# mmdagent/distantspeechrecognition-mirror

Hardware: AMD Instinct MI355X
Metric: decoded_audio_hours_per_sec (higher is better)
Workload: dtype f32

## Files before the change

### distantspeechrecognition-mirror_amd/csrc/k_viterbi.hip

```cpp
#include "common.h"
#include "wfst_graph.h"
#include "lattice.h"
#include "lexicon.h"
#include "wordtrace.h"
#include <algorithm>
#include <cmath>
#include <type_traits>

namespace dsr {

struct Tok { int32_t node; float ac; float lm; uint32_t bp; };
struct TokA { float ac; float lm; uint32_t bp; uint32_t xs; };
struct TokB { int32_t node; int32_t cnt; };
struct XRecD { int32_t dist; float cost; uint32_t meta; float eps1; int32_t dst; int32_t p2; int32_t dstXoff; int32_t dstCnt; };
struct Side { double ttl; float ac; float lm; int32_t rec; uint32_t prevBp; int32_t c; uint32_t next; };
struct CandA { double ttl; float ac; float lm; };
struct CandB { int32_t dst; int32_t next; int32_t rec; uint32_t prevBp; };
struct Bp { uint32_t prev; uint32_t rec; };

static constexpr uint32_t kNone = 0xFFFFFFFFu;
static constexpr uint32_t kEndBit = 0x80000000u;
static constexpr int kThreads = 1024;
static constexpr int kWaves = kThreads / 64;
static constexpr int kFastK = 8;
static constexpr int kB = 2;
static constexpr int kFastC = 24576;
static constexpr int kFastE = 8190;
static constexpr int kP1 = 16;
static constexpr int kW = 4;
static constexpr int kProfN = 48;
static constexpr int kSideLds = 496;

struct GraphDev {
  int nNodes, initial;
  const int* xoff; const XRec* xrec; const XRecD* xrecD; const int* xarc; const int* xpathOff;
  const int* eoff; const ERec* erec; const int* path; const float* pathCost;
  const float* arcCost; const uint32_t* arcOut; const uint32_t* arcIn;
  const int* nodeFinal; const float* nodeCost;
};

struct SegState { int n, status, maxActive, pad; long arenaOff, chunkEnd, arenaUsed; double thresh; long long stat[3]; };

struct DecDev {
  double beam, lmScale, lmPenalty, silPenalty; uint32_t silenceX; int noPen;
  int segFrames, segCount, segQueues, segDrop; long poolCap, poolChunk;    unsigned long long* poolNext; SegState* segState; int* segDone; TokA* saveA; TokB* saveB;
  int maxTok, maxCand; long arenaCap;
  TokA* tokA; TokB* tokB; TokA* ctok; Side* side; int fastOK; int* tokOff; int* tokCnt; int* owner; int* rank; int* chead; CandA* cA; CandB* cB; unsigned* first; unsigned* tags; Bp* arena;
  int* queue; long long* prof;
  int dumpOn; long dumpCap; long* dumpFrameOff; int* dumpNode; float* dumpAc; float* dumpLm; int* dumpArc; long* dumpCount;
  int latOn; long latCap; uint4* lat; double* latTtl; long* latFrameOff; int* arenaLat; int4* latFinal; int* latInfo;
  int topN; TokA* tokA3; TokB* tokB3;
};

struct VitArgs {
  GraphDev G; DecDev D;
  const float* scores; const int* nframesArr; int U, Tmax, nDist;
  dsr_decode_result* res; int* arcsOut; unsigned* wordsOut; int maxPath, useLdsRow, hashN, regionB, cntCap;
};
typedef const __attribute__((address_space(4))) VitArgs* KP;

__device__ __forceinline__ unsigned ld_u32(const unsigned* p) { return __hip_atomic_load(p, __ATOMIC_RELAXED, __HIP_MEMORY_SCOPE_AGENT); }
__device__ __forceinline__ int ld_i32(const int* p) { return __hip_atomic_load(p, __ATOMIC_RELAXED, __HIP_MEMORY_SCOPE_AGENT); }
__device__ __forceinline__ void st_u32(unsigned* p, unsigned v) { __hip_atomic_store(p, v, __ATOMIC_RELAXED, __HIP_MEMORY_SCOPE_AGENT); }
__device__ __forceinline__ void st_i32(int* p, int v) { __hip_atomic_store(p, v, __ATOMIC_RELAXED, __HIP_MEMORY_SCOPE_AGENT); }
__device__ __forceinline__ void st_u64_dev(void* p, unsigned long long v) { __hip_atomic_store(reinterpret_cast<unsigned long long*>(p), v, __ATOMIC_RELAXED, __HIP_MEMORY_SCOPE_AGENT); }
__device__ __forceinline__ unsigned long long ld_u64_dev(const void* p) { return __hip_atomic_load(reinterpret_cast<const unsigned long long*>(p), __ATOMIC_RELAXED, __HIP_MEMORY_SCOPE_AGENT); }

__device__ __forceinline__ int wave_incl_scan(int v, int )
{
  v += __builtin_amdgcn_update_dpp(0, v, 0x111, 0xF, 0xF, true);
  v += __builtin_amdgcn_update_dpp(0, v, 0x112, 0xF, 0xF, true);
  v += __builtin_amdgcn_update_dpp(0, v, 0x114, 0xF, 0xF, true);
// ... 101 lines not shown
  unsigned* const tab = hkey; const int tabN = NARROW ? 2 * hashN : hashN;
  Side* sideL = reinterpret_cast<Side*>(hfirst + hashN);
  unsigned short* cntL = reinterpret_cast<unsigned short*>(reinterpret_cast<unsigned char*>(hfirst + hashN) + regionB);
  __shared__ int s_waveTot[kWaves];
  __shared__ int s_waveTotE[kWaves];
  __shared__ double s_waveMin[kWaves];
  __shared__ float s_waveMag[kWaves];
  __shared__ unsigned long long s_waveKey[kWaves];
  __shared__ int s_sideN;
  __shared__ int s_tb[2];
  __shared__ unsigned s_bm[kFastC / 32];
  __shared__ unsigned s_gbase[kFastC / 64 + 4];
  __shared__ int s_cnt[(kFastK + 32) * kWaves];
  __shared__ int s_err;
  __shared__ long long s_prof[32]; __shared__ long long s_tlast;
  __shared__ long long s_hist[PROF ? 12 : 1]; __shared__ long long s_tfr;
  __shared__ long long s_stat[3];
  __shared__ int s_maxActive; __shared__ unsigned s_tag; __shared__ long long s_latOff;
  if (PROF && threadIdx.x < 32) s_prof[threadIdx.x] = 0;
  if (PROF && threadIdx.x < 12) s_hist[threadIdx.x] = 0;
#define TICK(ix) do { if (PROF && tid == 0) { const long long tn = (long long) wall_clock64(); s_prof[ix] += tn - s_tlast; s_tlast = tn; } } while (0)
  constexpr int nthr = kThreads, nw = kWaves;
  __shared__ int s_u, s_seg, s_help; __shared__ long long s_chunk;

  const int tid = threadIdx.x;
  const int slot = blockIdx.x;
#define TOKA(ix) ((EXTRA && (ix) == 2) ? ka->D.tokA3 + (size_t) slot * ka->D.maxTok : ka->D.tokA + ((size_t) slot * 2 + (size_t) (ix)) * ka->D.maxTok)
#define TOKB(ix) ((EXTRA && (ix) == 2) ? ka->D.tokB3 + (size_t) slot * ka->D.maxTok : ka->D.tokB + ((size_t) slot * 2 + (size_t) (ix)) * ka->D.maxTok)
#define curA TOKA(bufCur)
#define nxtA TOKA(bufNxt)
#define curB TOKB(bufCur)
#define nxtB TOKB(bufNxt)
#define sprA TOKA(bufSpr)
#define sprB TOKB(bufSpr)
#define ctok (ka->D.ctok + (size_t) slot * 8192)
// ... 85 lines not shown
      const int mode = (fr == T) ? 1 : 0;
      if (mode == 0 && useLdsRow) {
        if (preRow) {
          if (tid < nDist) srow[tid] = rowNext[0];
          if (tid + nthr < nDist) srow[tid + nthr] = rowNext[1];
          if (fr + 1 < T) {
            const float* nr = sc + (size_t) (fr + 1) * nDist;
            if (tid < nDist) rowNext[0] = nr[tid];
            if (tid + nthr < nDist) rowNext[1] = nr[tid + nthr];
          }
        } else { for (int i = tid; i < nDist; i += nthr) srow[i] = sc[(size_t) fr * nDist + i]; }
      }
      const float* rowG = sc + (size_t) fr * nDist;
      int numNew = 0, numStat = -1;
      if (fr > 0) TICK(23);
      if (PROF && tid == 0) { s_tlast = (long long) wall_clock64(); s_tfr = s_tlast; }
      bool fast = fastOK && mode == 0 && n <= fastCapN && !(EXTRA && (ka->D.latOn || ka->D.topN > 0));
      int Cfr = 0;

      if (fast) {
        const bool pre = preC >= 0;
        const int chunkT = ((n + nw * 64 - 1) / (nw * 64)) * 64;
        int C = preC, E = n;
        if (!pre) {
        float psc[kP1]; int pcn[kP1]; unsigned pk[kP1];
        int runC = 0, runE = 0;
        {
          const int b0 = wave * chunkT, b1 = (b0 + chunkT < n) ? b0 + chunkT : n;
#pragma unroll
          for (int g = 0; g < kP1; g += 8) {
            if (g * 64 < chunkT && cntOK) {
// ... 51 lines not shown
          for (int it = 0; it < kP1; it++) if (pk[it] & 0x80000000u) {
            const int e = ebase + (int) ((pk[it] >> 15) & 0xFFFFu); const int off = cbase + (int) (pk[it] & 0x7FFFu);
            if (!ident) ctok[e] = curA[wave * chunkT + it * 64 + lane];
            atomicOr(&s_bm[off >> 5], 1u << (off & 31));
            for (int g = (off >> 6) + 1; g <= ((off + pcn[it]) >> 6); g++) s_gbase[g] = (unsigned) (e + 1) | ((unsigned) (64 * g - off) << 13);
          }
          __syncthreads();
        }
        } else __syncthreads();
        if (C > fastCapC || E > eCap || C > regC) { fast = false; __syncthreads(); }
        else {
          RELOAD();
          const bool ident = (E == n);
          const TokA* __restrict__ ctk = ident ? curA : ctok;
          TICK(1);
          Cfr = C;
          RELOAD();
          int tq = tid; asm volatile("" : "+v"(tq)); const int lq = tq & 63, wq = tq >> 6;
          const int K = (C + nthr - 1) / nthr;
          float qac[kFastK], qlm[kFastK]; int qrec[kFastK]; unsigned ek[kFastK];
          double* const ttlS = reinterpret_cast<double*>(cA);
          uint4* const ovf = reinterpret_cast<uint4*>(cB);
          const XRecD* const xrecD = ka->G.xrecD; const float* const pathCost = ka->G.pathCost; const uint32_t silenceX = ka->D.silenceX;
          double locMin = HUGE_VAL; float locMag = 0.0f;
          const bool prevNull0 = (fr == 0);
          const double lmS = ka->D.lmScale, lsPen = __dmul_rn(ka->D.lmScale, ka->D.lmPenalty), lsSil = __dmul_rn(ka->D.lmScale, ka->D.silPenalty);
          const bool sil0 = (0u == silenceX);
#pragma unroll
          for (int k = 0; k < kFastK; k++) { qac[k] = 0.0f; qlm[k] = 0.0f; qrec[k] = 0; ek[k] = 0u; }

          const int nPass = (!NARROW && C > tableC) ? 2 : 1;
          auto table_insert = [&](const unsigned dst, const unsigned prod, const int c) __attribute__((always_inline)) -> unsigned {
            const unsigned key = dst + 1u;
// ... 402 lines not shown
            auto stage1 = [&](const int k, const float ac, const float lm, const int rec, const unsigned ekk) __attribute__((always_inline)) {
              const bool isFirst = (keepMask >> k) & 1ull;
              const unsigned long long bal = __ballot(isFirst);
              if (isFirst) stage[s_cnt[k * nw + wq] + __popcll(bal & ((1ull << lq) - 1ull))] = make_uint4(__float_as_uint(ac), __float_as_uint(lm), (unsigned) rec, ekk);
            };
#pragma unroll
            for (int k = 0; k < kFastK; k++) if (k < K) stage1(k, qac[k], qlm[k], qrec[k], ek[k]);
            for (int kb = kFastK; kb < K; kb += kB) {
              float oac[kB], olm[kB]; int orec[kB]; unsigned oek[kB]; park_load(kb, oac, olm, orec, oek);
#pragma unroll
              for (int i = 0; i < kB; i++) if (kb + i < K) stage1(kb + i, oac[i], olm[i], orec[i], oek[i]);
            }
            __syncthreads();
            TICK(21);
            const int q4 = hashN >> 2;
            const bool layNext = prune && numNew <= 2 * nthr;
            preC = -1;
            for (int f0 = 0; f0 < numNew; f0 += 2 * nthr) {
              uint4 en[2]; int4 dx[2]; uint32_t pv[2];
#pragma unroll
              for (int i = 0; i < 2; i++) {
                const int f = f0 + i * nthr + tq; const bool on = f < numNew;
                en[i] = stage[on ? f : 0];
                if (on) { unsigned wv = (NARROW || f < q4) ? 0u : 0xFFFFFFFFu; asm volatile("" : "+v"(wv)); stage[f] = make_uint4(wv, wv, wv, wv); }
              }
#pragma unroll
              for (int i = 0; i < 2; i++) {
                const bool on = f0 + i * nthr + tq < numNew;
                dx[i] = *at32<int4>(xrecW, (on ? (en[i].z & 0x3FFFFFFFu) : 0u) * 32u + 16u);
                const bool sw = on && (en[i].w & 0x80000000u) != 0u; const unsigned si = en[i].w & 0x7FFFFFFFu;
                const uint32_t* pb = (sw && si >= (unsigned) sideLds) ? &side[si].prevBp : &ctk[(sw || !on) ? 0u : (en[i].w & 0x1FFFu)].bp;
                pv[i] = *pb;
                if (sw && si < (unsigned) sideLds) pv[i] = sideL[si].prevBp;
              }
              if (layNext) {
                const int cA0 = (tq < numNew) ? dx[0].w : 0, cB0 = (nthr + tq < numNew) ? dx[1].w : 0;
                const int inA = wave_incl_scan(cA0, lq), inB = wave_incl_scan(cB0, lq);
                const bool bad = (tq < numNew && cA0 == 0) || (nthr + tq < numNew && cB0 == 0);
                const int badW = __any(bad) ? 1 : 0;
                if (lq == 63) { s_waveTot[wq] = inA; s_waveTotE[wq] = inB | (badW << 30); }
                __syncthreads();
                const int ta = (lq < nw) ? s_waveTot[lq] : 0, tbv = (lq < nw) ? s_waveTotE[lq] : 0, tb = tbv & 0x3FFFFFFF;
                const int sa = wave_incl_scan(ta, lq), sb = wave_incl_scan(tb, lq);
                const int totA = __builtin_amdgcn_readlane(sa, 63), totB = __builtin_amdgcn_readlane(sb, 63), wu = uni(wq);
                const int total = totA + totB;
                const int offA = total - (__builtin_amdgcn_readlane(sa - ta, wu) + inA), offB = total - (totA + __builtin_amdgcn_readlane(sb - tb, wu) + inB);
                const bool anyBad = __any((tbv >> 30) & 1);
#pragma unroll
                for (int i = 0; i < 2; i++) {
                  const int f = i * nthr + tq; const int off = i ? offB : offA, cn = i ? cB0 : cA0;
                  if (f < numNew && cn > 0) {
                    const int e = numNew - 1 - f;
                    atomicOr(&s_bm[off >> 5], 1u << (off & 31));
                    for (int g = (off >> 6) + 1; g <= ((off + cn) >> 6); g++) s_gbase[g] = (unsigned) (e + 1) | ((unsigned) (64 * g - off) << 13);
                  }
                }
                if (tq == 0) { s_sideN = 0; s_gbase[0] = 0; s_err = 0; }
                preC = anyBad ? -1 : total;
              }
#pragma unroll
              for (int i = 0; i < 2; i++) {
                const int f = f0 + i * nthr + tq;
                if (f < numNew) {
                  const int pos = numNew - 1 - f;
                  TokA na; na.ac = __uint_as_float(en[i].x); na.lm = __uint_as_float(en[i].y); na.bp = (uint32_t) (arenaOff + pos); na.xs = (uint32_t) dx[i].z | ((en[i].z & 0x40000000u) ? 0x80000000u : 0u);
                  TokB nb; nb.node = dx[i].x; nb.cnt = dx[i].w;
                  Bp bp; bp.prev = pv[i]; bp.rec = (uint32_t) (en[i].z & 0x3FFFFFFFu);
                  outA[pos] = na; outB[pos] = nb; outBp[pos] = bp;
                  if (pos < cntCap) cntL[pos] = (unsigned short) dx[i].w;
                }
              }
            }
            TICK(22);
          } else
          {
#pragma unroll
          for (int g4 = 0; g4 < kFastK; g4 += kW) if (g4 < K) write4(std::integral_constant<int, kW>{}, g4, &qac[g4], &qlm[g4], &qrec[g4], &ek[g4]);
          for (int kb = kFastK; kb < K; kb += kB) {
            float oac[kB], olm[kB]; int orec[kB]; unsigned oek[kB]; park_load(kb, oac, olm, orec, oek);
            write4(std::integral_constant<int, kB>{}, kb, oac, olm, orec, oek);
          }
          TICK(21);
          TICK(22);
          preC = -1;
          }
          cntOK = prune && numNew <= cntCap;
// ... 223 lines not shown
        }
      }
      if (EXTRA && ka->D.latOn) {
        uint4* lat = ka->D.lat + (size_t) u * ka->D.latCap; double* ltt = ka->D.latTtl + (size_t) u * ka->D.latCap;
        const long latOff = (long) s_latOff;
        for (int c = tid; c < C; c += nthr) {
          const CandA a = cA[c]; const CandB b = cB[c];
          lat[latOff + c] = make_uint4(__float_as_uint(a.ac), __float_as_uint(a.lm), (unsigned) b.rec, b.prevBp); ltt[latOff + c] = a.ttl;
        }
        __syncthreads();
        if (tid == 0) { s_latOff = latOff + C; ka->D.latFrameOff[(size_t) u * (ka->Tmax + 3) + fr + 1] = latOff + C; }
      }
      }
      __syncthreads();
      TICK(fast ? 7 : 8);
      if (PROF && tid == 0 && mode == 0) { const int cls = !fast ? 3 : Cfr <= kFastK * nthr ? 0 : Cfr <= 12288 ? 1 : 2; s_hist[cls] += 1; s_hist[4 + cls] += s_tlast - s_tfr; s_hist[8 + cls] += Cfr; }
      RELOAD();
      if (mode == 0) {
        if (dump) {
          long* cnt = ka->D.dumpCount; const long o = cnt[0];
          if (o + numNew <= ka->D.dumpCap) {
            for (int i = tid; i < numNew; i += nthr) {
              const TokA t = ld_tok(&nxtA[i]); ka->D.dumpNode[o + i] = nxtB[i].node; ka->D.dumpAc[o + i] = t.ac; ka->D.dumpLm[o + i] = t.lm;
              ka->D.dumpArc[o + i] = ka->G.xarc[arena[t.bp].rec];
            }
          }
          __syncthreads();
          if (tid == 0) { ka->D.dumpFrameOff[fr] = o; ka->D.dumpFrameOff[fr + 1] = o + numNew; cnt[0] = o + numNew; cnt[1] = fr + 1; }
        }
        if (numStat < 0) numStat = numNew;
        if (numStat == 0 || numNew == 0) { status = DSR_E_CONSISTENCY; break; }
// ... 105 lines not shown
      else __builtin_amdgcn_fence(__ATOMIC_RELEASE, "workgroup");
      __syncthreads();
      if (tid == 0) st_i32(&ka->D.segDone[u], seg + 1);
      continue;
    }
    if (status != DSR_OK) {
      if (tid == 0) {
        dsr_decode_result* const res = ka->res; clear_result(&res[u]); res[u].status = status; res[u].frames = T - 1;
        if (segS > 0) { st_i32(&ka->D.segState[u].status, status); asm volatile("s_waitcnt vmcnt(0)" ::: "memory"); st_i32(&ka->D.segDone[u], 0x7FFFFFFF); }
      }
    }
  }
  RELOAD();
  if (tid == 0) ka->D.tags[slot] = s_tag;
  if (PROF && tid < 32) ka->D.prof[slot * kProfN + tid] = s_prof[tid];
  if (PROF && tid < 12) ka->D.prof[slot * kProfN + 32 + tid] = s_hist[tid];
#undef TICK
#undef RELOAD
#undef TOKA
#undef TOKB
#undef curA
#undef nxtA
#undef curB
#undef nxtB
#undef sprA
#undef sprB
#undef ctok
#undef side
#undef cA
#undef cB
#undef arena
// ... 7 lines not shown
  DevBuf<int> d_xoff, d_xarc, d_xpathOff, d_eoff, d_path, d_nodeFinal, d_queue; DevBuf<float> d_pathCost;
  DevBuf<XRec> d_xrec; DevBuf<ERec> d_erec; DevBuf<float> d_arcCost, d_nodeCost; DevBuf<uint32_t> d_arcOut, d_arcIn;
  DevBuf<TokA> d_tokA, d_ctok; DevBuf<TokB> d_tokB; DevBuf<Side> d_side; DevBuf<XRecD> d_xrecD; int fastOK = 0; int maxCnt = 0; DevBuf<int> d_tokOff, d_tokCnt, d_owner, d_rank, d_chead; DevBuf<unsigned> d_tags; DevBuf<CandA> d_cA; DevBuf<CandB> d_cB; DevBuf<unsigned> d_first; DevBuf<Bp> d_arena;
  DevBuf<long long> d_prof; DevBuf<dsr_decode_result> d_res; DevBuf<int> d_arcs; DevBuf<unsigned> d_words;
  long arenaCap = 0; int initial = 0; unsigned tokenMemoryLimit = 0;
  long lastPoolCap = 0;
  DevBuf<SegState> d_segState; DevBuf<int> d_segDone; DevBuf<unsigned long long> d_poolNext; DevBuf<TokA> d_saveA; DevBuf<TokB> d_saveB;
  DevBuf<WTok> w_tok; DevBuf<WCand> w_cand; DevBuf<int> w_tokOff, w_rank; DevBuf<unsigned long long> w_best; DevBuf<unsigned> w_first; DevBuf<int4> w_traces; size_t w_tablesFor = 0;
  bool costNegZero = false; double costMinAbs = HUGE_VAL;
  DevBuf<uint4> d_lat; DevBuf<double> d_latTtl; DevBuf<long> d_latFrameOff; DevBuf<int> d_arenaLat; DevBuf<int4> d_latFinal; DevBuf<int> d_latInfo;
  int latU = 0, latTmax = 0; long latArenaCap = 0; WfstGraph graphCopy; DevBuf<TokA> d_tokA3; DevBuf<TokB> d_tokB3;
  const dsr_lexicon* lexIn = nullptr; const dsr_lexicon* lexOut = nullptr; uint32_t eosX = 0; std::string eosSymbol;
  int lastU = 0; size_t lastMaxPath = 0; bool lastPaths = false;
  PinBuf<dsr_decode_result> h_res; PinBuf<int> h_arcs; PinBuf<unsigned> h_words; hipEvent_t evDone = nullptr;
  int pendingU = 0; size_t pendingPath = 0; int pendingSlots = 0; long long* pendingProf = nullptr;
  int dumpOn = 0; long dumpCap = 0; DevBuf<long> d_dumpFrameOff, d_dumpCount; DevBuf<int> d_dumpNode, d_dumpArc; DevBuf<float> d_dumpAc, d_dumpLm;
  std::vector<int64_t> h_dumpFrameOff; std::vector<int32_t> h_dumpNode, h_dumpArc; std::vector<float> h_dumpAc, h_dumpLm; int64_t h_dumpFrames = 0;
};

}

using namespace dsr;
struct dsr_wfst : WfstGraph { dsr_lexicon* lexState = nullptr; dsr_lexicon* lexIn = nullptr; dsr_lexicon* lexOut = nullptr; };
struct dsr_decoder : DecoderState {};

extern "C" {

dsr_status dsr_wfst_create(dsr_wfst** out) { return guard([&] { if (!out) throw Error(DSR_E_PARAMETER, "null argument"); *out = new dsr_wfst(); }); }
dsr_status dsr_wfst_set_sorted_output(dsr_wfst* g, int on)
{ return guard([&] { if (!g) throw Error(DSR_E_PARAMETER, "null argument"); if (!g->arcs.empty()) throw Error(DSR_E_CONSISTENCY, "the transducer already has arcs"); g->sortedOutput = on != 0; }); }
// ... 260 lines not shown
      DSR_HIP(hipMemsetAsync(d->d_queue.p, 0, 8 * sizeof(int), st));
      WtArgs A; A.nNodes = d->nNodes; A.initial = d->initial; A.xoff = d->d_xoff.p; A.xrec = d->d_xrec.p; A.xarc = d->d_xarc.p; A.xpathOff = d->d_xpathOff.p; A.eoff = d->d_eoff.p;
      A.erec = d->d_erec.p; A.path = d->d_path.p; A.arcCost = d->d_arcCost.p; A.arcOut = d->d_arcOut.p; A.arcIn = d->d_arcIn.p; A.nodeFinal = d->d_nodeFinal.p; A.nodeCost = d->d_nodeCost.p;
      A.beam = c.beam; A.lmScale = c.lmScale; A.lmPenalty = c.lmPenalty; A.silPenalty = c.silPenalty; A.silenceX = c.silenceX; A.insertSilence = c.insertSilence;
      A.maxTok = c.maxActive; A.maxCand = c.maxCandidates; A.maxTraces = maxTraces;
      A.tok = d->w_tok.p; A.cand = d->w_cand.p; A.tokOff = d->w_tokOff.p; A.rank = d->w_rank.p; A.bestKey = d->w_best.p; A.firstSlot = d->w_first.p; A.traces = d->w_traces.p; A.queue = d->d_queue.p;
      A.scores = score; A.nframes = nframes; A.U = U; A.Tmax = Tmax; A.nDist = nDist; A.res = d->d_res.p; A.arcsOut = d->d_arcs.p; A.wordsOut = d->d_words.p; A.maxPath = maxPath;
      wordtrace_launch(A, slots, st);
      const size_t nPath = want_paths ? (size_t) U * maxPath : 0;
      d->h_res.reserve(U); d->h_arcs.reserve(nPath ? nPath : 1); d->h_words.reserve(nPath ? nPath : 1);
      DSR_HIP(hipMemcpyAsync(d->h_res.p, d->d_res.p, sizeof(dsr_decode_result) * U, hipMemcpyDeviceToHost, st));
      if (nPath) DSR_HIP(hipMemcpyAsync(d->h_arcs.p, d->d_arcs.p, sizeof(int) * nPath, hipMemcpyDeviceToHost, st));
      if (nPath) DSR_HIP(hipMemcpyAsync(d->h_words.p, d->d_words.p, sizeof(unsigned) * nPath, hipMemcpyDeviceToHost, st));
      if (!d->evDone) DSR_HIP(hipEventCreateWithFlags(&d->evDone, hipEventDisableTiming));
      DSR_HIP(hipEventRecord(d->evDone, st));
      d->pendingU = U; d->pendingPath = nPath; d->pendingSlots = slots; d->pendingProf = nullptr; d->latU = 0;
      return;
    }
    int32_t* arcs_out = want_paths ? (int32_t*) 1 : nullptr; uint32_t* words_out = want_paths ? (uint32_t*) 1 : nullptr;
    for (size_t a = 0; a < d->csr.in.size(); a++) if (d->csr.in[a] > (uint32_t) nDist) throw Error(DSR_E_INDEX, "arc input %u has no distribution (nDist=%d)", d->csr.in[a], nDist);
    int slots = d->cfg.streams; if (slots > U) slots = U; if (d->dumpOn) slots = 1;
    const bool latOn = d->cfg.latticeTokens > 0;
    if (latOn && d->dumpOn) throw Error(DSR_E_PARAMETER, "lattice bookkeeping and the token dump are separate debugging aids: enable one");
    int segFrames = 0;
    if (!latOn && !d->dumpOn && d->cfg.topN <= 0 && U > slots) {
      segFrames = getenv("DSR_VITERBI_SEG") ? atoi(getenv("DSR_VITERBI_SEG")) : 125;
      if (segFrames < 0 || 2 * segFrames > Tmax + 1) segFrames = 0;
      const double saveGB = (double) U * (double) d->cfg.maxActive * 24.0 / 1e9;
      if (saveGB > (getenv("DSR_VITERBI_SEG_SAVE_GB") ? atof(getenv("DSR_VITERBI_SEG_SAVE_GB")) : 16.0)) segFrames = 0;
    }
    int segQueues = 8;
// ... 26 lines not shown
    D.silenceX = d->cfg.silenceX; D.maxTok = d->cfg.maxActive; D.maxCand = d->cfg.maxCandidates; D.arenaCap = d->arenaCap;
    D.tokA = d->d_tokA.p; D.tokB = d->d_tokB.p; D.ctok = d->d_ctok.p; D.side = d->d_side.p; D.fastOK = d->fastOK; D.tokOff = d->d_tokOff.p; D.owner = d->d_owner.p; D.rank = d->d_rank.p; D.cA = d->d_cA.p; D.cB = d->d_cB.p;
    D.first = d->d_first.p; D.tags = d->d_tags.p; D.tokCnt = d->d_tokCnt.p; D.chead = d->d_chead.p; D.arena = d->d_arena.p; D.queue = d->d_queue.p;
    D.segDrop = getenv("DSR_VITERBI_SEG_DROP") ? (int) strtol(getenv("DSR_VITERBI_SEG_DROP"), nullptr, 0) : 0;
    D.segQueues = segQueues; D.segFrames = segFrames; D.segCount = segFrames > 0 ? (Tmax + segFrames) / segFrames : 1;
    D.poolCap = 0; D.poolChunk = 0; D.poolNext = nullptr; D.segState = nullptr; D.segDone = nullptr; D.saveA = nullptr; D.saveB = nullptr;
    if (segFrames > 0) {
      d->d_segState.reserve(U); d->d_segDone.reserve(U); d->d_poolNext.reserve(1);
      d->d_saveA.reserve((size_t) U * d->cfg.maxActive); d->d_saveB.reserve((size_t) U * d->cfg.maxActive);
      DSR_HIP(hipMemsetAsync(d->d_segDone.p, 0, sizeof(int) * (size_t) U, st)); DSR_HIP(hipMemsetAsync(d->d_poolNext.p, 0, sizeof(unsigned long long), st));
      D.poolCap = (long) ((size_t) std::max(poolArenas, slots) * (size_t) d->arenaCap); if (D.poolCap > (long) 0xFFFFFFF0L) D.poolCap = (long) 0xFFFFFFF0L;
      D.poolChunk = std::min<long>(262144, std::max<long>(4096, D.poolCap / (4 * (long) U)));
      D.poolNext = d->d_poolNext.p; D.segState = d->d_segState.p; D.segDone = d->d_segDone.p; D.saveA = d->d_saveA.p; D.saveB = d->d_saveB.p;
    }
    d->lastPoolCap = D.poolCap;
    D.prof = nullptr;
    if (getenv("DSR_VITERBI_PROF")) { d->d_prof.reserve((size_t) slots * kProfN); D.prof = d->d_prof.p; }
    D.dumpOn = d->dumpOn; D.dumpCap = d->dumpCap; D.dumpFrameOff = d->d_dumpFrameOff.p; D.dumpNode = d->d_dumpNode.p; D.dumpAc = d->d_dumpAc.p;
    D.dumpLm = d->d_dumpLm.p; D.dumpArc = d->d_dumpArc.p; D.dumpCount = d->d_dumpCount.p;
    D.topN = d->cfg.topN > 0 ? d->cfg.topN : 0; D.tokA3 = nullptr; D.tokB3 = nullptr;
    if (D.topN > 0) { d->d_tokA3.reserve((size_t) slots * d->cfg.maxActive); d->d_tokB3.reserve((size_t) slots * d->cfg.maxActive); D.tokA3 = d->d_tokA3.p; D.tokB3 = d->d_tokB3.p; }
    D.latOn = latOn ? 1 : 0; D.latCap = 0; D.lat = nullptr; D.latTtl = nullptr; D.latFrameOff = nullptr; D.arenaLat = nullptr; D.latFinal = nullptr; D.latInfo = nullptr;
    if (latOn) {
      const size_t cap = (size_t) d->cfg.latticeTokens;
      d->d_lat.reserve((size_t) U * cap); d->d_latTtl.reserve((size_t) U * cap); d->d_latFrameOff.reserve((size_t) U * (Tmax + 3));
      d->d_arenaLat.reserve((size_t) U * (size_t) d->arenaCap); d->d_latFinal.reserve((size_t) U * d->cfg.maxActive); d->d_latInfo.reserve((size_t) 4 * U);
      DSR_HIP(hipMemsetAsync(d->d_latInfo.p, 0, sizeof(int) * 4 * (size_t) U, st));
      D.latCap = (long) cap; D.lat = d->d_lat.p; D.latTtl = d->d_latTtl.p; D.latFrameOff = d->d_latFrameOff.p; D.arenaLat = d->d_arenaLat.p; D.latFinal = d->d_latFinal.p; D.latInfo = d->d_latInfo.p;
      d->latU = U; d->latTmax = Tmax; d->latArenaCap = d->arenaCap;
    } else d->latU = 0;
// ... 5 lines not shown
    int useLds = (size_t) nDist * sizeof(float) <= 64 * 1024;
    if (useLds && (size_t) ((nDist + 3) & ~3) * sizeof(float) + (size_t) hashMax * 8 + eoffB > ldsCap) useLds = 0;
    const size_t rowB = useLds ? (size_t) ((nDist + 3) & ~3) * sizeof(float) : 16;
    int hashN = hashMax; while (hashN > 0 && rowB + (size_t) hashN * 8 + eoffB > ldsCap) hashN >>= 1;
    if (getenv("DSR_VITERBI_NOHASH")) hashN = 0;
    int cntCap = (hashN > 0 && d->maxCnt < 65536 && rowB + (size_t) hashN * 8 + eoffB + 4096 <= ldsCap) ? 2048 : 0;
    if (getenv("DSR_VITERBI_NOCNT")) cntCap = 0;
    const size_t lds = rowB + (size_t) hashN * 8 + eoffB + 2 * (size_t) cntCap;
    const char* const tableEnv = getenv("DSR_VITERBI_TABLE");
    const bool narrow = d->nNodes <= 65535 && hashN == hashMax && !(tableEnv && !strcmp(tableEnv, "wide"));
    if (narrow) modes |= 4;
    if (getenv("DSR_VITERBI_SEG_VERBOSE")) fprintf(stderr, "[dsr viterbi] %d utterances on %d workgroups: %s, %s state table\n", U, slots, segFrames > 0 ? (segQueues == 8 ? "time-sliced, XCD-bound queues" : "time-sliced, one queue") : "run to completion", narrow ? "narrow" : "wide");
    VitArgs A; A.G = G; A.D = D; A.scores = score; A.nframesArr = nframes; A.U = U; A.Tmax = Tmax; A.nDist = nDist; A.res = d->d_res.p;
    A.arcsOut = (arcs_out || words_out) ? d->d_arcs.p : nullptr; A.wordsOut = (arcs_out || words_out) ? d->d_words.p : nullptr; A.maxPath = maxPath;
    A.useLdsRow = useLds; A.hashN = hashN; A.regionB = (int) eoffB; A.cntCap = cntCap;
#define DSR_LAUNCH_V(MM) { DSR_HIP(hipFuncSetAttribute((const void*) k_viterbi<MM>, hipFuncAttributeMaxDynamicSharedMemorySize, (int) lds)); \
      hipLaunchKernelGGL(k_viterbi<MM>, dim3(slots), dim3(kThreads), lds, st, A); }
    switch (modes) { case 0: DSR_LAUNCH_V(0) break; case 1: DSR_LAUNCH_V(1) break; case 2: DSR_LAUNCH_V(2) break; case 3: DSR_LAUNCH_V(3) break;
                     case 4: DSR_LAUNCH_V(4) break; case 5: DSR_LAUNCH_V(5) break; case 6: DSR_LAUNCH_V(6) break; default: DSR_LAUNCH_V(7) break; }
#undef DSR_LAUNCH_V
    DSR_HIP(hipGetLastError());
    const size_t nPath = want_paths ? (size_t) U * maxPath : 0;
    d->h_res.reserve(U); d->h_arcs.reserve(nPath ? nPath : 1); d->h_words.reserve(nPath ? nPath : 1);
    DSR_HIP(hipMemcpyAsync(d->h_res.p, d->d_res.p, sizeof(dsr_decode_result) * U, hipMemcpyDeviceToHost, st));
    if (nPath) DSR_HIP(hipMemcpyAsync(d->h_arcs.p, d->d_arcs.p, sizeof(int) * nPath, hipMemcpyDeviceToHost, st));
    if (nPath) DSR_HIP(hipMemcpyAsync(d->h_words.p, d->d_words.p, sizeof(unsigned) * nPath, hipMemcpyDeviceToHost, st));
    if (!d->evDone) DSR_HIP(hipEventCreateWithFlags(&d->evDone, hipEventDisableTiming));
    DSR_HIP(hipEventRecord(d->evDone, st));
    d->pendingU = U; d->pendingPath = nPath; d->pendingSlots = slots; d->pendingProf = D.prof;
  });
}

dsr_status dsr_decoder_decode_collect(dsr_decoder* d, dsr_decode_result* res, int32_t* arcs_out, uint32_t* words_out)
{
  return guard([&] {
    if (!d || !res) throw Error(DSR_E_PARAMETER, "null argument");
    if (d->pendingU <= 0) throw Error(DSR_E_CONSISTENCY, "no decode in flight");
    const int U = d->pendingU; const size_t nPath = d->pendingPath; const int slots = d->pendingSlots; long long* prof = d->pendingProf;
    d->pendingU = 0; d->lastU = U; d->lastPaths = nPath > 0; d->lastMaxPath = nPath > 0 ? nPath / (size_t) U : 0;
    DSR_HIP(hipEventSynchronize(d->evDone));
    memcpy(res, d->h_res.p, sizeof(dsr_decode_result) * U);
    if (arcs_out && nPath) memcpy(arcs_out, d->h_arcs.p, sizeof(int) * nPath);
    if (words_out && nPath) memcpy(words_out, d->h_words.p, sizeof(unsigned) * nPath);
    if (getenv("DSR_VITERBI_SEG_VERBOSE") && d->d_poolNext.p && d->lastPoolCap > 0) {
      unsigned long long used = 0; DSR_HIP(hipMemcpy(&used, d->d_poolNext.p, sizeof(used), hipMemcpyDeviceToHost));
      fprintf(stderr, "[dsr viterbi] pool of back-pointer records: %.1f M of %.1f M taken\n", used / 1e6, d->lastPoolCap / 1e6);
    }
    if (prof) {
      std::vector<long long> hp((size_t) slots * kProfN); DSR_HIP(hipMemcpy(hp.data(), prof, hp.size() * sizeof(long long), hipMemcpyDeviceToHost));
      double acc[32] = {0}; for (int s2 = 0; s2 < slots; s2++) for (int i = 0; i < 32; i++) acc[i] += (double) hp[(size_t) s2 * kProfN + i];
      fprintf(stderr, "[dsr viterbi prof] mean us per slot:");
      for (int i = 0; i < 32; i++) if (i != 15) fprintf(stderr, " p%d=%.0f", i, acc[i] / slots / 100.0);
      fprintf(stderr, "\n");
      double tmin = 1e30, tmax = 0.0, tsum = 0.0;
      for (int s2 = 0; s2 < slots; s2++) { double t = 0.0; for (int i = 0; i < 32; i++) if (i != 15) t += (double) hp[(size_t) s2 * kProfN + i]; t /= 100.0; tsum += t; if (t < tmin) tmin = t; if (t > tmax) tmax = t; }
      {
        double h[12] = {0}; for (int s2 = 0; s2 < slots; s2++) for (int i = 0; i < 12; i++) h[i] += (double) hp[(size_t) s2 * kProfN + 32 + i];
        const double nf = h[0] + h[1] + h[2] + h[3], tk = h[4] + h[5] + h[6] + h[7];
        static const char* const cn[4] = {"<=8192", "<=12288", ">12288", "memory path"};
        for (int c = 0; c < 4; c++) if (h[c] > 0) fprintf(stderr, "[dsr viterbi prof] frames with %s placements: %.1f %% of the frames, %.1f %% of the frame time, %.1f us per frame, %.2f ns per placement\n",
                                                          cn[c], 100.0 * h[c] / nf, 100.0 * h[4 + c] / tk, h[4 + c] / 100.0 / h[c], h[4 + c] * 10.0 / h[8 + c]);
      }
      fprintf(stderr, "[dsr viterbi prof] busy us per slot: mean %.0f min %.0f max %.0f\n", tsum / slots, tmin, tmax);
      if (slots >= 64 && slots % 8 == 0) {
        double bx[8] = {0}; for (int s2 = 0; s2 < slots; s2++) { double t = 0.0; for (int i = 0; i < 32; i++) if (i != 15) t += (double) hp[(size_t) s2 * kProfN + i]; bx[s2 & 7] += t / 100.0; }
        fprintf(stderr, "[dsr viterbi prof] busy us per slot, by XCD:"); for (int q = 0; q < 8; q++) fprintf(stderr, " %.0f", bx[q] / (slots / 8)); fprintf(stderr, "\n");
      }
    }
    if (d->dumpOn) {
      long cnt[2]; DSR_HIP(hipMemcpy(cnt, d->d_dumpCount.p, sizeof(cnt), hipMemcpyDeviceToHost));
      const long N = cnt[0] < d->dumpCap ? cnt[0] : d->dumpCap; d->h_dumpFrames = cnt[1];
      std::vector<long> fo(cnt[1] + 1); if (cnt[1] > 0) DSR_HIP(hipMemcpy(fo.data(), d->d_dumpFrameOff.p, sizeof(long) * (cnt[1] + 1), hipMemcpyDeviceToHost));
      d->h_dumpFrameOff.assign(fo.begin(), fo.end());
      d->h_dumpNode.resize(N); d->h_dumpArc.resize(N); d->h_dumpAc.resize(N); d->h_dumpLm.resize(N);
      if (N > 0) {
        DSR_HIP(hipMemcpy(d->h_dumpNode.data(), d->d_dumpNode.p, sizeof(int) * N, hipMemcpyDeviceToHost));
        DSR_HIP(hipMemcpy(d->h_dumpArc.data(), d->d_dumpArc.p, sizeof(int) * N, hipMemcpyDeviceToHost));
        DSR_HIP(hipMemcpy(d->h_dumpAc.data(), d->d_dumpAc.p, sizeof(float) * N, hipMemcpyDeviceToHost));
        DSR_HIP(hipMemcpy(d->h_dumpLm.data(), d->d_dumpLm.p, sizeof(float) * N, hipMemcpyDeviceToHost));
      }
    }
  });
}

dsr_status dsr_decoder_decode_batch(dsr_decoder* d, const float* score, const int32_t* nframes, int U, int Tmax, int nDist,
                                    dsr_decode_result* res, int32_t* arcs_out, uint32_t* words_out, int maxPath, void* stream)
{
  if (!res) return guard([&] { throw Error(DSR_E_PARAMETER, "null argument"); });
  if (U <= 0) return DSR_OK;
  const dsr_status s1 = dsr_decoder_decode_launch(d, score, nframes, U, Tmax, nDist, maxPath, (arcs_out || words_out) ? 1 : 0, stream);
  if (s1 != DSR_OK) return s1;
  return dsr_decoder_decode_collect(d, res, arcs_out, words_out);
}

namespace {
struct LatHost {
  std::vector<long> frameOff; std::vector<dsr::LatPlace> place; std::vector<double> ttl; std::vector<dsr::LatBp> arena; std::vector<int> arenaLat; std::vector<dsr::LatFinalTok> fin;
  dsr::LatInput in;
// ... 112 lines not shown
```

### distantspeechrecognition-mirror_amd/dsr/_capi.py

```python
import ctypes as C
import os
import re

C_ = C

import numpy as np

_HERE = os.path.dirname(os.path.abspath(__file__))
_LIBPATH = os.path.join(os.path.dirname(_HERE), "lib", "libdsr_hip.so")
_lib = None

vp, i32, i64, f32, f64, u32 = C.c_void_p, C.c_int32, C.c_int64, C.c_float, C.c_double, C.c_uint32

ERROR_NAMES = ["OK", "JERROR", "JALLOCATION", "JARITHMETIC", "JCONSISTENCY", "JDIMENSION", "JINDEX", "JINITIALIZATION",
               "JIO", "JITERATOR", "JPYTHON", "JKEY", "JNUMERIC", "JPARAMETER", "JPARSE", "JTYPE"]
E_ITERATOR, E_IO, E_INDEX, E_DIMENSION = 9, 8, 6, 5
E_CONSISTENCY, E_KEY, E_PARAMETER, E_PARSE = 4, 11, 13, 14


class DsrError(Exception):

    def __init__(self, status, msg):
        super().__init__("%s: %s" % (ERROR_NAMES[status] if 0 <= status < len(ERROR_NAMES) else status, msg))
        self.status = status
# ... 1800 lines not shown
        if nframes is None:
            nframes = torch.full((U,), T, dtype=torch.int32, device=scores.device)
        if maxPath is None:
            maxPath = 4 * T + 64
        res = (DecodeResult * U)()
        arcs = np.zeros((U, maxPath), np.int32); words = np.zeros((U, maxPath), np.uint32)
        check(_lib.dsr_decoder_decode_batch(self.h, _dev(scores), _dev(nframes), U, T, nDist, C.byref(res), _ptr(arcs), _ptr(words), maxPath, cur_stream()))
        out = []
        for u in range(U):
            r = res[u]
            out.append(dict(status=r.status, score=r.score, ac=r.ac, lm=r.lm, frames=r.frames, reachedFinal=bool(r.reachedFinal),
                            arcs=arcs[u, :min(r.nArcs, maxPath)].copy(), words=words[u, :min(r.nWords, maxPath)].copy(),
                            activeHypos=r.activeHypos, maxActive=r.maxActiveSeen, placements=r.placements, registerFrames=r.registerFrames, finalStatesN=r.finalStatesN))
        return out

    def lattice(self, u=0, eosX=0):
        h = vp(); check(_lib.dsr_decoder_lattice(self.h, int(u), int(eosX), C.byref(h)))
        return Lattice(h)

    def writeGMM(self, u, conv, channel, spk, utt, cfrom, score, fileName="", frameInterval=0.01):
        check(_lib.dsr_decoder_write_gmm(self.h, int(u), conv.encode(), channel.encode(), spk.encode(), utt.encode(), float(cfrom), float(score),
                                         (fileName or "").encode(), float(frameInterval)))

    def get_dump(self):
        n = i64(); fo = C.POINTER(i64)(); nd = C.POINTER(i32)(); ac = C.POINTER(f32)(); lm = C.POINTER(f32)(); arc = C.POINTER(i32)()
        check(_lib.dsr_decoder_get_dump(self.h, C.byref(n), C.byref(fo), C.byref(nd), C.byref(ac), C.byref(lm), C.byref(arc)))
        nf = n.value
        off = np.array([fo[i] for i in range(nf + 1)], np.int64) if nf > 0 else np.zeros(1, np.int64)
        N = int(off[-1])
        g = lambda p, dt: np.ctypeslib.as_array(p, (N,)).astype(dt).copy() if N > 0 else np.zeros(0, dt)
# ... 328 lines not shown
```

### include/dsr.h

```cpp
#ifndef DSR_H
#define DSR_H
#include <stddef.h>
#include <stdint.h>

#ifdef __cplusplus
extern "C" {
#endif

typedef int dsr_status;
enum {
  DSR_OK = 0,
  DSR_E_ERROR = 1,
  DSR_E_ALLOCATION = 2,
  DSR_E_ARITHMETIC = 3,
  DSR_E_CONSISTENCY = 4,
  DSR_E_DIMENSION = 5,
  DSR_E_INDEX = 6,
  DSR_E_INITIALIZATION = 7,
  DSR_E_IO = 8,
  DSR_E_ITERATOR = 9,
  DSR_E_PYTHON = 10,
  DSR_E_KEY = 11,
  DSR_E_NUMERIC = 12,
  DSR_E_PARAMETER = 13,
// ... 417 lines not shown
  int32_t nWords;
  int32_t status;
  int32_t maxActiveSeen;
  int64_t activeHypos;
  int64_t placements;
  int64_t registerFrames;
  int32_t finalStatesN;
  int32_t reserved_;
} dsr_decode_result;
dsr_status dsr_decoder_decode_batch(dsr_decoder*, const float* score_dev, const int32_t* nframes_dev, int U,
                                    int Tmax, int nDist, dsr_decode_result* res, int32_t* arcs_out,
                                    uint32_t* words_out, int maxPath, void* stream);
dsr_status dsr_decoder_decode_launch(dsr_decoder*, const float* score_dev, const int32_t* nframes_dev, int U,
                                     int Tmax, int nDist, int maxPath, int want_paths, void* stream);
dsr_status dsr_decoder_decode_collect(dsr_decoder*, dsr_decode_result* res, int32_t* arcs_out, uint32_t* words_out);
typedef struct dsr_lattice dsr_lattice;
dsr_status dsr_decoder_lattice(dsr_decoder*, int u, uint32_t eosX, dsr_lattice** out);
dsr_status dsr_decoder_write_gmm(dsr_decoder*, int u, const char* conv, const char* channel, const char* spk, const char* utt, double cfrom, double score,
                                 const char* fileName, double frameInterval);
void       dsr_lattice_destroy(dsr_lattice*);
int        dsr_lattice_num_nodes(const dsr_lattice*);
int        dsr_lattice_num_edges(const dsr_lattice*);
int        dsr_lattice_final_states_n(const dsr_lattice*);
dsr_status dsr_lattice_get(const dsr_lattice*, int32_t* nodeFinal, int32_t* from, int32_t* to, uint32_t* in, uint32_t* out, int32_t* start,
                           int32_t* end, double* ac, double* lm);
dsr_status dsr_lattice_write(dsr_lattice*, const char* fileName, int writeData);
dsr_status dsr_lattice_read(const char* fileName, int noSelfLoops, int readData, dsr_lexicon* inputLex, dsr_lexicon* outputLex, dsr_lattice** out);
dsr_status dsr_lattice_rescore(dsr_lattice*, double lmScale, double lmPenalty, double silPenalty, unsigned silenceX, float* score);
dsr_status dsr_lattice_best_hypo(const dsr_lattice*, int useInputSymbols, uint32_t* symbols, int cap, int* n);
dsr_status dsr_lattice_gamma_probs(dsr_lattice*, double acScale, double lmScale, double lmPenalty, double silPenalty, unsigned silenceX, double* logProb);
// ... 442 lines not shown
```

Measured before the change: 26.26.

## Lay out next-frame placements over multiple rounds instead of a single round

```diff
diff --git a/distantspeechrecognition-mirror_amd/csrc/k_viterbi.hip b/distantspeechrecognition-mirror_amd/csrc/k_viterbi.hip
--- a/distantspeechrecognition-mirror_amd/csrc/k_viterbi.hip
+++ b/distantspeechrecognition-mirror_amd/csrc/k_viterbi.hip
@@ -28,7 +28,7 @@
 static constexpr int kFastE = 8190;
 static constexpr int kP1 = 16;
 static constexpr int kW = 4;
-static constexpr int kProfN = 48;
+static constexpr int kProfN = 52;
 static constexpr int kSideLds = 496;
 
 struct GraphDev {
@@ -47,6 +47,7 @@
   int maxTok, maxCand; long arenaCap;
   TokA* tokA; TokB* tokB; TokA* ctok; Side* side; int fastOK; int* tokOff; int* tokCnt; int* owner; int* rank; int* chead; CandA* cA; CandB* cB; unsigned* first; unsigned* tags; Bp* arena;
   int* queue; long long* prof;
+  unsigned long long* layStat;
   int dumpOn; long dumpCap; long* dumpFrameOff; int* dumpNode; float* dumpAc; float* dumpLm; int* dumpArc; long* dumpCount;
   int latOn; long latCap; uint4* lat; double* latTtl; long* latFrameOff; int* arenaLat; int4* latFinal; int* latInfo;
   int topN; TokA* tokA3; TokB* tokB3;
@@ -56,6 +57,7 @@
   GraphDev G; DecDev D;
   const float* scores; const int* nframesArr; int U, Tmax, nDist;
   dsr_decode_result* res; int* arcsOut; unsigned* wordsOut; int maxPath, useLdsRow, hashN, regionB, cntCap;
+  int lay1;
 };
 typedef const __attribute__((address_space(4))) VitArgs* KP;
 
@@ -187,11 +189,13 @@
   __shared__ int s_cnt[(kFastK + 32) * kWaves];
   __shared__ int s_err;
   __shared__ long long s_prof[32]; __shared__ long long s_tlast;
-  __shared__ long long s_hist[PROF ? 12 : 1]; __shared__ long long s_tfr;
+  __shared__ long long s_hist[PROF ? 20 : 1]; __shared__ long long s_tfr; __shared__ long long s_p12;
   __shared__ long long s_stat[3];
   __shared__ int s_maxActive; __shared__ unsigned s_tag; __shared__ long long s_latOff;
+  __shared__ long long s_lay[4];
+  if (threadIdx.x < 4) s_lay[threadIdx.x] = 0;
   if (PROF && threadIdx.x < 32) s_prof[threadIdx.x] = 0;
-  if (PROF && threadIdx.x < 12) s_hist[threadIdx.x] = 0;
+  if (PROF && threadIdx.x < 20) s_hist[threadIdx.x] = 0;
 #define TICK(ix) do { if (PROF && tid == 0) { const long long tn = (long long) wall_clock64(); s_prof[ix] += tn - s_tlast; s_tlast = tn; } } while (0)
   constexpr int nthr = kThreads, nw = kWaves;
   __shared__ int s_u, s_seg, s_help; __shared__ long long s_chunk;
@@ -307,7 +311,7 @@
       const float* rowG = sc + (size_t) fr * nDist;
       int numNew = 0, numStat = -1;
       if (fr > 0) TICK(23);
-      if (PROF && tid == 0) { s_tlast = (long long) wall_clock64(); s_tfr = s_tlast; }
+      if (PROF && tid == 0) { s_tlast = (long long) wall_clock64(); s_tfr = s_tlast; s_p12 = -1; }
       bool fast = fastOK && mode == 0 && n <= fastCapN && !(EXTRA && (ka->D.latOn || ka->D.topN > 0));
       int Cfr = 0;
 
@@ -389,9 +393,11 @@
           const bool ident = (E == n);
           const TokA* __restrict__ ctk = ident ? curA : ctok;
           TICK(1);
+          if (PROF && tid == 0 && !pre) s_p12 = s_tlast - s_tfr;
           Cfr = C;
           RELOAD();
           int tq = tid; asm volatile("" : "+v"(tq)); const int lq = tq & 63, wq = tq >> 6;
+          if (tq == nthr - 1) { s_lay[pre ? 0 : 1] += 1; if (C > kFastK * nthr) { s_lay[2] += C - kFastK * nthr; if (pre) s_lay[3] += 1; } }
           const int K = (C + nthr - 1) / nthr;
           float qac[kFastK], qlm[kFastK]; int qrec[kFastK]; unsigned ek[kFastK];
           double* const ttlS = reinterpret_cast<double*>(cA);
@@ -824,9 +830,10 @@
             __syncthreads();
             TICK(21);
             const int q4 = hashN >> 2;
-            const bool layNext = prune && numNew <= 2 * nthr;
+            const bool layNext = prune && (ka->lay1 ? numNew <= 2 * nthr : numNew <= eCap);
             preC = -1;
-            for (int f0 = 0; f0 < numNew; f0 += 2 * nthr) {
+            int laid = 0; bool layBad = false;
+            for (int f0 = numNew > 0 ? ((numNew - 1) / (2 * nthr)) * (2 * nthr) : -1; f0 >= 0; f0 -= 2 * nthr) {
               uint4 en[2]; int4 dx[2]; uint32_t pv[2];
 #pragma unroll
               for (int i = 0; i < 2; i++) {
@@ -844,29 +851,30 @@
                 if (sw && si < (unsigned) sideLds) pv[i] = sideL[si].prevBp;
               }
               if (layNext) {
-                const int cA0 = (tq < numNew) ? dx[0].w : 0, cB0 = (nthr + tq < numNew) ? dx[1].w : 0;
+                const int cA0 = (f0 + tq < numNew) ? dx[0].w : 0, cB0 = (f0 + nthr + tq < numNew) ? dx[1].w : 0;
                 const int inA = wave_incl_scan(cA0, lq), inB = wave_incl_scan(cB0, lq);
-                const bool bad = (tq < numNew && cA0 == 0) || (nthr + tq < numNew && cB0 == 0);
+                const bool bad = (f0 + tq < numNew && cA0 == 0) || (f0 + nthr + tq < numNew && cB0 == 0);
                 const int badW = __any(bad) ? 1 : 0;
-                if (lq == 63) { s_waveTot[wq] = inA; s_waveTotE[wq] = inB | (badW << 30); }
+                const bool odd = ((f0 / (2 * nthr)) & 1) != 0;
+                int* const xA = odd ? reinterpret_cast<int*>(s_waveKey) : s_waveTot; int* const xB = odd ? reinterpret_cast<int*>(s_waveKey) + kWaves : s_waveTotE;
+                if (lq == 63) { xA[wq] = inA; xB[wq] = inB | (badW << 30); }
                 __syncthreads();
-                const int ta = (lq < nw) ? s_waveTot[lq] : 0, tbv = (lq < nw) ? s_waveTotE[lq] : 0, tb = tbv & 0x3FFFFFFF;
+                const int ta = (lq < nw) ? xA[lq] : 0, tbv = (lq < nw) ? xB[lq] : 0, tb = tbv & 0x3FFFFFFF;
                 const int sa = wave_incl_scan(ta, lq), sb = wave_incl_scan(tb, lq);
                 const int totA = __builtin_amdgcn_readlane(sa, 63), totB = __builtin_amdgcn_readlane(sb, 63), wu = uni(wq);
                 const int total = totA + totB;
-                const int offA = total - (__builtin_amdgcn_readlane(sa - ta, wu) + inA), offB = total - (totA + __builtin_amdgcn_readlane(sb - tb, wu) + inB);
-                const bool anyBad = __any((tbv >> 30) & 1);
+                const int offA = laid + total - (__builtin_amdgcn_readlane(sa - ta, wu) + inA), offB = laid + total - (totA + __builtin_amdgcn_readlane(sb - tb, wu) + inB);
+                if (__any((tbv >> 30) & 1)) layBad = true;
 #pragma unroll
                 for (int i = 0; i < 2; i++) {
-                  const int f = i * nthr + tq; const int off = i ? offB : offA, cn = i ? cB0 : cA0;
-                  if (f < numNew && cn > 0) {
+                  const int f = f0 + i * nthr + tq; const int off = i ? offB : offA, cn = i ? cB0 : cA0;
+                  if (f < numNew && cn > 0 && off + cn <= fastCapC) {
                     const int e = numNew - 1 - f;
                     atomicOr(&s_bm[off >> 5], 1u << (off & 31));
                     for (int g = (off >> 6) + 1; g <= ((off + cn) >> 6); g++) s_gbase[g] = (unsigned) (e + 1) | ((unsigned) (64 * g - off) << 13);
                   }
                 }
-                if (tq == 0) { s_sideN = 0; s_gbase[0] = 0; s_err = 0; }
-                preC = anyBad ? -1 : total;
+                laid += total;
               }
 #pragma unroll
               for (int i = 0; i < 2; i++) {
@@ -880,6 +888,10 @@
                   if (pos < cntCap) cntL[pos] = (unsigned short) dx[i].w;
                 }
               }
+            }
+            if (layNext) {
+              if (tq == 0) { s_sideN = 0; s_gbase[0] = 0; s_err = 0; }
+              preC = (layBad || laid > fastCapC || laid > regC) ? -1 : laid;
             }
             TICK(22);
           } else
@@ -1133,7 +1145,7 @@
       }
       __syncthreads();
       TICK(fast ? 7 : 8);
-      if (PROF && tid == 0 && mode == 0) { const int cls = !fast ? 3 : Cfr <= kFastK * nthr ? 0 : Cfr <= 12288 ? 1 : 2; s_hist[cls] += 1; s_hist[4 + cls] += s_tlast - s_tfr; s_hist[8 + cls] += Cfr; }
+      if (PROF && tid == 0 && mode == 0) { const int cls = !fast ? 3 : Cfr <= kFastK * nthr ? 0 : Cfr <= 12288 ? 1 : 2; s_hist[cls] += 1; s_hist[4 + cls] += s_tlast - s_tfr; s_hist[8 + cls] += Cfr; if (s_p12 >= 0) { s_hist[12 + cls] += s_p12; s_hist[16 + cls] += 1; } }
       RELOAD();
       if (mode == 0) {
         if (dump) {
@@ -1269,7 +1281,8 @@
   RELOAD();
   if (tid == 0) ka->D.tags[slot] = s_tag;
   if (PROF && tid < 32) ka->D.prof[slot * kProfN + tid] = s_prof[tid];
-  if (PROF && tid < 12) ka->D.prof[slot * kProfN + 32 + tid] = s_hist[tid];
+  if (PROF && tid < 20) ka->D.prof[slot * kProfN + 32 + tid] = s_hist[tid];
+  if (tid < 4 && s_lay[tid]) atomicAdd(&ka->D.layStat[tid], (unsigned long long) s_lay[tid]);
 #undef TICK
 #undef RELOAD
 #undef TOKA
@@ -1307,6 +1320,7 @@
   int lastU = 0; size_t lastMaxPath = 0; bool lastPaths = false;
   PinBuf<dsr_decode_result> h_res; PinBuf<int> h_arcs; PinBuf<unsigned> h_words; hipEvent_t evDone = nullptr;
   int pendingU = 0; size_t pendingPath = 0; int pendingSlots = 0; long long* pendingProf = nullptr;
+  DevBuf<unsigned long long> d_layStat; PinBuf<unsigned long long> h_layStat; bool pendingLay = false; long long lastLay[4] = {0, 0, 0, 0};
   int dumpOn = 0; long dumpCap = 0; DevBuf<long> d_dumpFrameOff, d_dumpCount; DevBuf<int> d_dumpNode, d_dumpArc; DevBuf<float> d_dumpAc, d_dumpLm;
   std::vector<int64_t> h_dumpFrameOff; std::vector<int32_t> h_dumpNode, h_dumpArc; std::vector<float> h_dumpAc, h_dumpLm; int64_t h_dumpFrames = 0;
 };
@@ -1597,7 +1611,7 @@
       if (nPath) DSR_HIP(hipMemcpyAsync(d->h_words.p, d->d_words.p, sizeof(unsigned) * nPath, hipMemcpyDeviceToHost, st));
       if (!d->evDone) DSR_HIP(hipEventCreateWithFlags(&d->evDone, hipEventDisableTiming));
       DSR_HIP(hipEventRecord(d->evDone, st));
-      d->pendingU = U; d->pendingPath = nPath; d->pendingSlots = slots; d->pendingProf = nullptr; d->latU = 0;
+      d->pendingU = U; d->pendingPath = nPath; d->pendingSlots = slots; d->pendingProf = nullptr; d->pendingLay = false; d->latU = 0;
       return;
     }
     int32_t* arcs_out = want_paths ? (int32_t*) 1 : nullptr; uint32_t* words_out = want_paths ? (uint32_t*) 1 : nullptr;
@@ -1654,6 +1668,8 @@
       D.poolNext = d->d_poolNext.p; D.segState = d->d_segState.p; D.segDone = d->d_segDone.p; D.saveA = d->d_saveA.p; D.saveB = d->d_saveB.p;
     }
     d->lastPoolCap = D.poolCap;
+    d->d_layStat.reserve(4); d->h_layStat.reserve(4); D.layStat = d->d_layStat.p;
+    DSR_HIP(hipMemsetAsync(d->d_layStat.p, 0, 4 * sizeof(unsigned long long), st));
     D.prof = nullptr;
     if (getenv("DSR_VITERBI_PROF")) { d->d_prof.reserve((size_t) slots * kProfN); D.prof = d->d_prof.p; }
     D.dumpOn = d->dumpOn; D.dumpCap = d->dumpCap; D.dumpFrameOff = d->d_dumpFrameOff.p; D.dumpNode = d->d_dumpNode.p; D.dumpAc = d->d_dumpAc.p;
@@ -1689,6 +1705,7 @@
     VitArgs A; A.G = G; A.D = D; A.scores = score; A.nframesArr = nframes; A.U = U; A.Tmax = Tmax; A.nDist = nDist; A.res = d->d_res.p;
     A.arcsOut = (arcs_out || words_out) ? d->d_arcs.p : nullptr; A.wordsOut = (arcs_out || words_out) ? d->d_words.p : nullptr; A.maxPath = maxPath;
     A.useLdsRow = useLds; A.hashN = hashN; A.regionB = (int) eoffB; A.cntCap = cntCap;
+    { const char* const layEnv = getenv("DSR_VITERBI_LAY"); A.lay1 = (layEnv && !strcmp(layEnv, "1round")) ? 1 : 0; }
 #define DSR_LAUNCH_V(MM) { DSR_HIP(hipFuncSetAttribute((const void*) k_viterbi<MM>, hipFuncAttributeMaxDynamicSharedMemorySize, (int) lds)); \
       hipLaunchKernelGGL(k_viterbi<MM>, dim3(slots), dim3(kThreads), lds, st, A); }
     switch (modes) { case 0: DSR_LAUNCH_V(0) break; case 1: DSR_LAUNCH_V(1) break; case 2: DSR_LAUNCH_V(2) break; case 3: DSR_LAUNCH_V(3) break;
@@ -1700,9 +1717,10 @@
     DSR_HIP(hipMemcpyAsync(d->h_res.p, d->d_res.p, sizeof(dsr_decode_result) * U, hipMemcpyDeviceToHost, st));
     if (nPath) DSR_HIP(hipMemcpyAsync(d->h_arcs.p, d->d_arcs.p, sizeof(int) * nPath, hipMemcpyDeviceToHost, st));
     if (nPath) DSR_HIP(hipMemcpyAsync(d->h_words.p, d->d_words.p, sizeof(unsigned) * nPath, hipMemcpyDeviceToHost, st));
+    DSR_HIP(hipMemcpyAsync(d->h_layStat.p, d->d_layStat.p, 4 * sizeof(unsigned long long), hipMemcpyDeviceToHost, st));
     if (!d->evDone) DSR_HIP(hipEventCreateWithFlags(&d->evDone, hipEventDisableTiming));
     DSR_HIP(hipEventRecord(d->evDone, st));
-    d->pendingU = U; d->pendingPath = nPath; d->pendingSlots = slots; d->pendingProf = D.prof;
+    d->pendingU = U; d->pendingPath = nPath; d->pendingSlots = slots; d->pendingProf = D.prof; d->pendingLay = true;
   });
 }
 
@@ -1717,6 +1735,7 @@
     memcpy(res, d->h_res.p, sizeof(dsr_decode_result) * U);
     if (arcs_out && nPath) memcpy(arcs_out, d->h_arcs.p, sizeof(int) * nPath);
     if (words_out && nPath) memcpy(words_out, d->h_words.p, sizeof(unsigned) * nPath);
+    for (int i = 0; i < 4; i++) d->lastLay[i] = d->pendingLay ? (long long) d->h_layStat.p[i] : 0;
     if (getenv("DSR_VITERBI_SEG_VERBOSE") && d->d_poolNext.p && d->lastPoolCap > 0) {
       unsigned long long used = 0; DSR_HIP(hipMemcpy(&used, d->d_poolNext.p, sizeof(used), hipMemcpyDeviceToHost));
       fprintf(stderr, "[dsr viterbi] pool of back-pointer records: %.1f M of %.1f M taken\n", used / 1e6, d->lastPoolCap / 1e6);
@@ -1730,11 +1749,15 @@
       double tmin = 1e30, tmax = 0.0, tsum = 0.0;
       for (int s2 = 0; s2 < slots; s2++) { double t = 0.0; for (int i = 0; i < 32; i++) if (i != 15) t += (double) hp[(size_t) s2 * kProfN + i]; t /= 100.0; tsum += t; if (t < tmin) tmin = t; if (t > tmax) tmax = t; }
       {
-        double h[12] = {0}; for (int s2 = 0; s2 < slots; s2++) for (int i = 0; i < 12; i++) h[i] += (double) hp[(size_t) s2 * kProfN + 32 + i];
+        double h[20] = {0}; for (int s2 = 0; s2 < slots; s2++) for (int i = 0; i < 20; i++) h[i] += (double) hp[(size_t) s2 * kProfN + 32 + i];
         const double nf = h[0] + h[1] + h[2] + h[3], tk = h[4] + h[5] + h[6] + h[7];
         static const char* const cn[4] = {"<=8192", "<=12288", ">12288", "memory path"};
         for (int c = 0; c < 4; c++) if (h[c] > 0) fprintf(stderr, "[dsr viterbi prof] frames with %s placements: %.1f %% of the frames, %.1f %% of the frame time, %.1f us per frame, %.2f ns per placement\n",
                                                           cn[c], 100.0 * h[c] / nf, 100.0 * h[4 + c] / tk, h[4 + c] / 100.0 / h[c], h[4 + c] * 10.0 / h[8 + c]);
+        for (int c = 0; c < 3; c++) if (h[16 + c] > 0) fprintf(stderr, "[dsr viterbi prof] frames with %s placements on the general layout: %.1f %% of the class, P1 + P2 %.2f us per such frame\n",
+                                                               cn[c], 100.0 * h[16 + c] / h[c], h[12 + c] / 100.0 / h[16 + c]);
+        fprintf(stderr, "[dsr viterbi prof] register-path frames laid out by the frame before %lld (with parked placements %lld), on the general layout %lld; parked placements %lld\n",
+                d->lastLay[0], d->lastLay[3], d->lastLay[1], d->lastLay[2]);
       }
       fprintf(stderr, "[dsr viterbi prof] busy us per slot: mean %.0f min %.0f max %.0f\n", tsum / slots, tmin, tmax);
       if (slots >= 64 && slots % 8 == 0) {
@@ -1757,6 +1780,9 @@
     }
   });
 }
+
+dsr_status dsr_decoder_last_stats(const dsr_decoder* d, int64_t* out4)
+{ return guard([&] { if (!d || !out4) throw Error(DSR_E_PARAMETER, "null argument"); for (int i = 0; i < 4; i++) out4[i] = (int64_t) d->lastLay[i]; }); }
 
 dsr_status dsr_decoder_decode_batch(dsr_decoder* d, const float* score, const int32_t* nframes, int U, int Tmax, int nDist,
                                     dsr_decode_result* res, int32_t* arcs_out, uint32_t* words_out, int maxPath, void* stream)
diff --git a/distantspeechrecognition-mirror_amd/dsr/_capi.py b/distantspeechrecognition-mirror_amd/dsr/_capi.py
--- a/distantspeechrecognition-mirror_amd/dsr/_capi.py
+++ b/distantspeechrecognition-mirror_amd/dsr/_capi.py
@@ -1838,6 +1838,10 @@
                             activeHypos=r.activeHypos, maxActive=r.maxActiveSeen, placements=r.placements, registerFrames=r.registerFrames, finalStatesN=r.finalStatesN))
         return out
 
+    def last_stats(self):
+        v = (i64 * 4)(); check(_lib.dsr_decoder_last_stats(self.h, v))
+        return dict(preLaid=int(v[0]), general=int(v[1]), parked=int(v[2]), preLaidLarge=int(v[3]))
+
     def lattice(self, u=0, eosX=0):
         h = vp(); check(_lib.dsr_decoder_lattice(self.h, int(u), int(eosX), C.byref(h)))
         return Lattice(h)
diff --git a/include/dsr.h b/include/dsr.h
--- a/include/dsr.h
+++ b/include/dsr.h
@@ -455,6 +455,7 @@
 dsr_status dsr_decoder_decode_launch(dsr_decoder*, const float* score_dev, const int32_t* nframes_dev, int U,
                                      int Tmax, int nDist, int maxPath, int want_paths, void* stream);
 dsr_status dsr_decoder_decode_collect(dsr_decoder*, dsr_decode_result* res, int32_t* arcs_out, uint32_t* words_out);
+dsr_status dsr_decoder_last_stats(const dsr_decoder*, int64_t* out4);
 typedef struct dsr_lattice dsr_lattice;
 dsr_status dsr_decoder_lattice(dsr_decoder*, int u, uint32_t eosX, dsr_lattice** out);
 dsr_status dsr_decoder_write_gmm(dsr_decoder*, int u, const char* conv, const char* channel, const char* spk, const char* utt, double cfrom, double score,
```

Measured after the change: 26.46, median of 6. Within noise of the previous version (+0.8%).
